# Boese0601/MagicDance

Measured on NVIDIA H100. Metric: denoise-steps/sec @512x512 50-step DDIM, higher is better.
Workload: dtype f16

## Files before the change

include/magicdance_b200.h:

```cpp
#ifndef MAGICDANCE_B200_H_
#define MAGICDANCE_B200_H_

#include <stdint.h>

#ifdef __cplusplus
extern "C" {
#endif

#define MDB_OK 0
#define MDB_ERR_INVALID (-1)
#define MDB_ERR_CUDA (-2)
#define MDB_ERR_UNSUPPORTED (-3)

#define MDB_ABI_VERSION 2

typedef void* mdb_stream_t;

int mdb_abi_version(void);
const char* mdb_last_error(void);
int mdb_device_check(void);
int64_t mdb_launch_count(void);
int64_t mdb_abi_struct_bytes(int32_t which);

#define MDB_TUNE_GEMM_PAIR_MIN_TILES 1
#define MDB_TUNE_ATTN40_2Q_MIN_CTAS 3
#define MDB_TUNE_GEMM_BN80_BELOW 4
enum {
  MDB_TUNE_GEMM_SKINNY_CTAS = 5,
  MDB_TUNE_GEMM_SPLIT_MIN_CHUNKS = 6
};
int mdb_set_tuning(int32_t key, int32_t value);
int32_t mdb_get_tuning(int32_t key);

#define MDB_EPI_NONE 0
#define MDB_EPI_GEGLU 1

typedef struct mdb_gemm_desc {
  const void* a;
  int64_t lda;
  const void* a2;
  int64_t lda2;
  int32_t k1;
  int32_t conv;
  int32_t nb, h, w, c;
  const void* b;
  int64_t ldb;
  void* d;
  int64_t ldd;
  const float* bias;
  int64_t bias_batch_stride;
  int32_t rows_per_batch;
  int32_t epilogue;
  const void* residual;
  int64_t ldr;
  int32_t m, n, k;
  int32_t splits;
  float* splitk_ws;
  const float* ln_u;
  float ln_eps;
} mdb_gemm_desc;

int mdb_gemm_f16(const mdb_gemm_desc* desc, mdb_stream_t stream);
// ... 148 lines not shown
```

magicdance_b200/_lib.py:

```python
from __future__ import annotations

import ctypes as C
import os

from . import build as _build

c_void_p, c_int32, c_int64, c_float = C.c_void_p, C.c_int32, C.c_int64, C.c_float


class GemmDesc(C.Structure):
    _fields_ = [
        ("a", c_void_p), ("lda", c_int64), ("a2", c_void_p), ("lda2", c_int64),
        ("k1", c_int32), ("conv", c_int32), ("nb", c_int32), ("h", c_int32), ("w", c_int32), ("c", c_int32),
        ("b", c_void_p), ("ldb", c_int64), ("d", c_void_p), ("ldd", c_int64),
        ("bias", c_void_p), ("bias_batch_stride", c_int64), ("rows_per_batch", c_int32), ("epilogue", c_int32),
        ("residual", c_void_p), ("ldr", c_int64),
        ("m", c_int32), ("n", c_int32), ("k", c_int32), ("splits", c_int32), ("splitk_ws", c_void_p),
        ("ln_u", c_void_p), ("ln_eps", c_float),
    ]


class AttnDesc(C.Structure):
    _fields_ = [
        ("q", c_void_p), ("ldq", c_int64),
# ... 102 lines not shown
    "mdb_layernorm_f16": (c_int32, [c_void_p, c_void_p, c_void_p, c_void_p, c_int64, c_int32, c_float, c_void_p]),
    "mdb_groupnorm_bwd_f16": (c_int32, [C.POINTER(GroupNormBwdDesc), c_void_p]),
    "mdb_groupnorm_bwd_ws_floats": (c_int64, [C.POINTER(GroupNormBwdDesc)]),
    "mdb_layernorm_bwd_f16": (c_int32, [C.POINTER(LayerNormBwdDesc), c_void_p]),
    "mdb_layernorm_bwd_ws_floats": (c_int64, [C.POINTER(LayerNormBwdDesc)]),
    "mdb_geglu_f16": (c_int32, [c_void_p, c_int64, c_void_p, c_int64, c_int64, c_int32, c_void_p]),
    "mdb_geglu_bwd_f16": (c_int32, [c_void_p, c_int64, c_void_p, c_int64, c_void_p, c_int64, c_int64, c_int32,
                                    c_void_p]),
    "mdb_conv3x3_direct_f16": (c_int32, [c_void_p, c_void_p, c_void_p, c_void_p, c_void_p, c_int32, c_int32, c_int32,
                                         c_int32, c_int32, c_int32, c_int32, c_void_p]),
    "mdb_conv3x3_direct_bwd_f16": (c_int32, [C.POINTER(Conv3x3BwdDesc), c_void_p]),
    "mdb_conv3x3_direct_bwd_ws_floats": (c_int64, [C.POINTER(Conv3x3BwdDesc)]),
    "mdb_im2col3x3_f16": (c_int32, [c_void_p, c_void_p, c_int32, c_int32, c_int32, c_int32, c_int32, c_void_p]),
    "mdb_im2col3x3_br_f16": (c_int32, [c_void_p, c_void_p, c_int32, c_int32, c_int32, c_int32, c_int32, c_void_p]),
    "mdb_upsample2x_f16": (c_int32, [c_void_p, c_void_p, c_int32, c_int32, c_int32, c_int32, c_void_p]),
    "mdb_upsample2x_bwd_f16": (c_int32, [c_void_p, c_void_p, c_int32, c_int32, c_int32, c_int32, c_int32, c_int32,
                                         c_void_p]),
    "mdb_add_f16": (c_int32, [c_void_p, c_void_p, c_void_p, c_int64, c_int32, c_int32, c_void_p]),
    "mdb_timestep_embedding_f32": (c_int32, [c_void_p, c_int32, c_void_p, c_int32, c_int32, c_void_p]),
    "mdb_skinny_linear_f32": (c_int32, [c_void_p, c_void_p, c_void_p, c_void_p, c_int32, c_int32, c_int32, c_int32,
                                        c_int32, c_void_p]),
    "mdb_skinny_linear_bwd_f32": (c_int32, [C.POINTER(SkinnyBwdDesc), c_void_p]),
    "mdb_skinny_linear_bwd_ws_floats": (c_int64, [C.POINTER(SkinnyBwdDesc)]),
    "mdb_nchw_f32_to_nhwc_f16": (c_int32, [c_void_p, c_void_p, c_int32, c_int32, c_int32, c_int32, c_int32, c_void_p]),
    "mdb_nhwc_f16_to_nchw_f32": (c_int32, [c_void_p, c_void_p, c_int32, c_int32, c_int32, c_int32, c_void_p]),
    "mdb_softmax_rows_f16": (c_int32, [c_void_p, c_int64, c_int32, c_int32, c_float, c_void_p]),
    "mdb_cfg_ddim_update_f32": (c_int32, [c_void_p, c_void_p, c_void_p, c_void_p, c_void_p, c_void_p, c_int64,
                                          c_void_p, c_int32, c_void_p]),
}

_lib = None
ABI_VERSION = 2
TUNE_GEMM_PAIR_MIN_TILES, TUNE_ATTN40_2Q_MIN_CTAS, TUNE_GEMM_BN80_BELOW = 1, 3, 4
TUNE_GEMM_SKINNY_CTAS, TUNE_GEMM_SPLIT_MIN_CHUNKS = 5, 6


def library_path() -> str:
    return os.environ.get("MAGICDANCE_B200_LIB", _build.LIB_PATH)


def load():
    global _lib
    if _lib is not None:
        return _lib
    path = library_path()
    if not os.path.isfile(path):
        raise RuntimeError(
            f"magicdance_b200: kernel library {path} is missing — run `python -m magicdance_b200.build` "
            "(there is no CPU/PyTorch fallback for the hot path)")
    if path == _build.LIB_PATH and os.path.isdir(_build.CSRC) and not _build.is_fresh():
        raise RuntimeError(f"magicdance_b200: {path} was not built from the sources in {_build.CSRC} "
                           "(stamp mismatch) — run `python -m magicdance_b200.build`")
    lib = C.CDLL(path)
    for name, (res, args) in SIGNATURES.items():
        fn = getattr(lib, name)
        fn.restype = res
        fn.argtypes = args
    if lib.mdb_abi_version() != ABI_VERSION:
        raise RuntimeError(f"magicdance_b200: ABI version mismatch ({lib.mdb_abi_version()} != {ABI_VERSION}); "
                           "rebuild the library")
    for which, mirror in ((0, GemmDesc), (1, AttnDesc), (2, AttnBwdDesc), (3, GemmBwdDesc), (4, GroupNormBwdDesc),
                          (5, LayerNormBwdDesc), (6, Conv3x3BwdDesc), (7, SkinnyBwdDesc)):
        if lib.mdb_abi_struct_bytes(which) != C.sizeof(mirror):
            raise RuntimeError(f"magicdance_b200: {mirror.__name__} mirrors {C.sizeof(mirror)} bytes, the library's "
                               f"struct has {lib.mdb_abi_struct_bytes(which)}: the binding and the library disagree")
    _lib = lib
    return lib
# ... 7 lines not shown
```

magicdance_b200/csrc/attention.cu:

```cuda
#include <stdlib.h>

#include <type_traits>

#include "common.cuh"

namespace mdb {

constexpr int kBQ = 128;

template <int D, int BKV, int STAGES>
struct AttnCfg {
  static constexpr int kDkChunks = (D + 63) / 64;
  static constexpr int kDV = (D + 15) / 16 * 16;
  static constexpr int kKSteps = kDV / 16;
  static constexpr int kQBytes = kDkChunks * kBQ * 128;
  static constexpr int kKBytes = kDkChunks * BKV * 128;
  static constexpr int kVBytes = kDV * 128;
  static constexpr int kStageBytes = kKBytes + kVBytes;
  static constexpr int kSmem = kQBytes + STAGES * kStageBytes + 1024;
  static_assert(BKV == 64, "one 128-byte swizzle row of keys per V^T tile");
  static_assert(kVBytes % 1024 == 0 && kKBytes % 1024 == 0, "stage tiles start on swizzle-atom boundaries");
};

struct AttnKParams {
// ... 142 lines not shown
    for (int h = 0; h < 2; ++h) {
      float l = l_run[h];
      l += __shfl_xor_sync(0xffffffffu, l, 1);
      l += __shfl_xor_sync(0xffffffffu, l, 2);
      inv_l[h] = 1.0f / l;
      l_row[h] = l;
    }
    const int r = wg * 64 + (warp & 3) * 16 + (lane >> 2);
    if constexpr (LSE) {
      if ((lane & 3) == 0) {
#pragma unroll
        for (int h = 0; h < 2; ++h) {
          const int q = q0 + r + 8 * h;
          if (q < p.nq)
            p.lse[(static_cast<long long>(b) * gridDim.y + head) * p.nq + q] =
                (m_run[h] + log2f(l_row[h])) * 0.6931471805599453f;
        }
      }
    }
#pragma unroll
    for (int h = 0; h < 2; ++h) {
      const int q = q0 + r + 8 * h;
      if (q < p.nq) {
        __half* op = p.out + (static_cast<long long>(b) * p.nq + q) * p.ldo + head * D + cq;
#pragma unroll
        for (int c8 = 0; c8 < D / 8; ++c8)
          *reinterpret_cast<uint32_t*>(op + 8 * c8) =
              pack_half2(o[4 * c8 + 2 * h] * inv_l[h], o[4 * c8 + 2 * h + 1] * inv_l[h]);
      }
    }
  }
}

static int g_attn40_2q_min_ctas = 512;
int get_attn_tuning() { return g_attn40_2q_min_ctas; }
void set_attn_tuning(int v) { g_attn40_2q_min_ctas = v; }

template <int D, int BKV, int STAGES, int MINB, bool LSE = false, typename P>
static int launch_attn(const P& kp, dim3 grid, cudaStream_t st) {
  using C = AttnCfg<D, BKV, STAGES>;
  static_assert(MINB == 1 || C::kSmem <= 113 * 1024, "two CTAs per SM must fit");
  constexpr auto kern = attn_wg_kernel<D, BKV, STAGES, MINB, LSE>;
  if (int rc = set_max_dyn_smem<kern>(C::kSmem)) return rc;
  MDB_CHECK_CUDA(launch_pdl(kern, grid, dim3(kWsThreads), C::kSmem, st, kp));
  count_launch();
  return MDB_OK;
}

template <int D, int BKV>
static int build_and_launch(const mdb_attn_desc* a, float* lse, cudaStream_t st) {
  constexpr int kDV = AttnCfg<D, BKV, 1>::kDV;
  AttnKParams kp;
  memset(&kp, 0, sizeof(kp));
  const int hd = a->heads * a->d;
  int rc;
  if ((rc = tmap_heads(&kp.tmQ, a->q, a->d, a->heads, (uint64_t)a->batch * a->nq, a->ldq, kBQ))) return rc;
  auto mk_kv = [&](const void* k, long long ldk, const void* vt, long long ldvt, int n, int nb, int ldvb,
                   CUtensorMap* tk, CUtensorMap* tv) -> int {
    int r = tmap_heads(tk, k, a->d, a->heads, (uint64_t)nb * n, ldk, BKV);
    if (r) return r;
    return tmap_vt(tv, vt, n, nb, ldvb, hd, ldvt, kDV);
  };
  if ((rc = mk_kv(a->k0, a->ldk0, a->vt0, a->ldvt0, a->n0, a->kv0_batches, a->ldv0_batch, &kp.tmK0, &kp.tmV0))) return rc;
  if (a->n1 > 0) {
    if ((rc = mk_kv(a->k1, a->ldk1, a->vt1, a->ldvt1, a->n1, a->kv1_batches, a->ldv1_batch, &kp.tmK1, &kp.tmV1)))
      return rc;
  }
  kp.out = static_cast<__half*>(a->out);
  kp.ldo = a->ldo;
  kp.nq = a->nq;
  kp.n0 = a->n0;
  kp.n1 = a->n1;
  kp.kv0_batches = a->kv0_batches;
  kp.kv1_batches = a->kv1_batches;
  kp.bank_batches = a->n1 > 0 ? a->bank_batches : 0;
  kp.scale_log2 = a->scale * 1.4426950408889634f;
  dim3 grid((a->nq + kBQ - 1) / kBQ, a->heads, a->batch);
  if (lse != nullptr) {
    AttnLseKParams lp;
    memset(&lp, 0, sizeof(lp));
    static_cast<AttnKParams&>(lp) = kp;
    lp.lse = lse;
    if constexpr (D == 40) {
      const long long ctas = (long long)grid.x * grid.y * grid.z;
      if (ctas >= (long long)g_attn40_2q_min_ctas) return launch_attn<D, BKV, 3, 2, true>(lp, grid, st);
    }
    return launch_attn<D, BKV, (D == 160 ? 2 : 4), 1, true>(lp, grid, st);
  }
  if constexpr (D == 40) {
    const long long ctas = (long long)grid.x * grid.y * grid.z;
    if (ctas >= (long long)g_attn40_2q_min_ctas) return launch_attn<D, BKV, 3, 2>(kp, grid, st);
  }
  return launch_attn<D, BKV, (D == 160 ? 2 : 4), 1>(kp, grid, st);
}

static int attention_entry(const mdb_attn_desc* a, float* lse, cudaStream_t st) {
  switch (a->d) {
    case 40:
      return build_and_launch<40, 64>(a, lse, st);
    case 80:
      return build_and_launch<80, 64>(a, lse, st);
    case 160:
      return build_and_launch<160, 64>(a, lse, st);
    default:
      set_error("mdb_attention_f16: head dim %d not supported (40, 80, 160)", a->d);
      return MDB_ERR_UNSUPPORTED;
  }
}

int attention_check_desc(const mdb_attn_desc* a) {
  MDB_REQUIRE(a != nullptr, "mdb_attention_f16: null descriptor");
  MDB_REQUIRE(a->q && a->k0 && a->vt0 && a->out, "mdb_attention_f16: null operand");
  MDB_REQUIRE(a->batch > 0 && a->heads > 0 && a->nq > 0 && a->n0 > 0 && a->n1 >= 0,
              "mdb_attention_f16: bad shape");
  MDB_REQUIRE(a->n1 == 0 || (a->k1 && a->vt1), "mdb_attention_f16: n1 > 0 needs k1/vt1");
  MDB_REQUIRE(a->kv0_batches == 1 || a->kv0_batches == a->batch, "mdb_attention_f16: kv0_batches must be 1 or batch");
  MDB_REQUIRE(a->n1 == 0 || a->kv1_batches == 1 || a->kv1_batches >= a->bank_batches,
              "mdb_attention_f16: kv1_batches must be 1 or cover bank_batches");
  MDB_REQUIRE(a->ldv0_batch >= a->n0 && a->ldv0_batch % 8 == 0, "mdb_attention_f16: ldv0_batch must be >= n0 and %% 8");
  MDB_REQUIRE(a->n1 == 0 || (a->ldv1_batch >= a->n1 && a->ldv1_batch % 8 == 0),
              "mdb_attention_f16: ldv1_batch must be >= n1 and %% 8");
  MDB_REQUIRE(a->ldo % 8 == 0 && (reinterpret_cast<uintptr_t>(a->out) & 15) == 0, "mdb_attention_f16: out alignment");
// ... 20 lines not shown
```

magicdance_b200/csrc/common.cuh:

```cuda
#pragma once

#include <cuda.h>
#include <cuda_fp16.h>
#include <cuda_runtime.h>
#include <cudaTypedefs.h>
#include <stdint.h>
#include <stdio.h>
#include <string.h>

#include "../../include/magicdance_b200.h"
#include "wgmma.cuh"

namespace mdb {

void set_error(const char* fmt, ...);

#define MDB_CHECK_CUDA(expr)                                                                     \
  do {                                                                                           \
    cudaError_t _e = (expr);                                                                     \
    if (_e != cudaSuccess) {                                                                     \
      mdb::set_error("%s:%d: %s failed: %s", __FILE__, __LINE__, #expr, cudaGetErrorString(_e)); \
      return MDB_ERR_CUDA;                                                                       \
    }                                                                                            \
  } while (0)

#define MDB_REQUIRE(cond, ...)      \
  do {                              \
    if (!(cond)) {                  \
      mdb::set_error(__VA_ARGS__);  \
      return MDB_ERR_INVALID;       \
    }                               \
  } while (0)

void count_launch(int n = 1);
int get_gemm_tuning(int key);
void set_gemm_tuning(int key, int value);
int get_attn_tuning();
void set_attn_tuning(int v);

constexpr int kNumSms = 132;

int tmap_rows(CUtensorMap* out, const void* base, uint64_t inner, uint64_t rows, long long ld, uint32_t box_inner,
              uint32_t box_rows);
int tmap_heads(CUtensorMap* out, const void* base, int d, int heads, uint64_t tokens, long long ld,
               uint32_t box_tokens);
int tmap_vt(CUtensorMap* out, const void* base, int n, int nb, long long ldvb, int rows, long long ldvt,
            uint32_t box_rows);
int tmap_nhwc(CUtensorMap* out, const void* base, int c, int w, int h, int nb, long long ld, const uint32_t box[4],
              int cs);
int tmap_nhwc_im2col(CUtensorMap* out, const void* base, int c, int w, int h, int nb, long long ld, int pixels,
                     int cs);

enum { kBoxOk, kBoxWideRows, kBoxRowsPerTile, kBoxImagesPerTile, kBoxTooLarge };
int pixel_box(int ho, int wo, int cs, int rows, bool fwd, uint32_t box[4]);

#ifdef __CUDACC__

bool pdl_enabled();
template <typename... KArgs, typename... Args>
inline cudaError_t launch_pdl_cluster2(void (*kernel)(KArgs...), dim3 grid, dim3 block, size_t smem,
                                       cudaStream_t stream, unsigned cluster_x, unsigned cluster_z, Args&&... args) {
  cudaLaunchConfig_t cfg;
  memset(&cfg, 0, sizeof(cfg));
  cfg.gridDim = grid;
  cfg.blockDim = block;
  cfg.dynamicSmemBytes = smem;
  cfg.stream = stream;
  cudaLaunchAttribute attr[2];
  int n = 0;
  if (cluster_z > 1 || cluster_x > 1) {
    attr[n].id = cudaLaunchAttributeClusterDimension;
// ... 255 lines not shown
```

magicdance_b200/csrc/misc.cu:

```cuda
#include <stdarg.h>
#include <stdlib.h>

#include <atomic>

#include "common.cuh"

namespace mdb {

static thread_local char g_err[512] = "";
static std::atomic<long long> g_launches{0};

void set_error(const char* fmt, ...) {
  va_list ap;
  va_start(ap, fmt);
  vsnprintf(g_err, sizeof(g_err), fmt, ap);
  va_end(ap);
}
void count_launch(int n) { g_launches.fetch_add(n, std::memory_order_relaxed); }
bool pdl_enabled() { return true; }

static PFN_cuTensorMapEncodeTiled_v12000 g_encode = nullptr;

static int make_tmap_f16(CUtensorMap* out, const void* base, int rank, const uint64_t* dims,
                         const uint64_t* strides_bytes, const uint32_t* box, const uint32_t* elem_strides = nullptr) {
// ... 524 lines not shown

extern "C" int64_t mdb_abi_struct_bytes(int32_t which) {
  switch (which) {
    case 0:
      return (int64_t)sizeof(mdb_gemm_desc);
    case 1:
      return (int64_t)sizeof(mdb_attn_desc);
    case 2:
      return (int64_t)sizeof(mdb_attn_bwd_desc);
    case 3:
      return (int64_t)sizeof(mdb_gemm_bwd_desc);
    case 4:
      return (int64_t)sizeof(mdb_groupnorm_bwd_desc);
    case 5:
      return (int64_t)sizeof(mdb_layernorm_bwd_desc);
    case 6:
      return (int64_t)sizeof(mdb_conv3x3_bwd_desc);
    case 7:
      return (int64_t)sizeof(mdb_skinny_linear_bwd_desc);
    default:
      return -1;
  }
}

extern "C" int mdb_set_tuning(int32_t key, int32_t value) {
  switch (key) {
    case MDB_TUNE_GEMM_PAIR_MIN_TILES:
    case MDB_TUNE_GEMM_BN80_BELOW:
    case MDB_TUNE_GEMM_SKINNY_CTAS:
    case MDB_TUNE_GEMM_SPLIT_MIN_CHUNKS:
      mdb::set_gemm_tuning(key, value);
      return MDB_OK;
    case MDB_TUNE_ATTN40_2Q_MIN_CTAS:
      mdb::set_attn_tuning(value);
      return MDB_OK;
    default:
      mdb::set_error("mdb_set_tuning: unknown key %d", key);
      return MDB_ERR_INVALID;
  }
}

extern "C" int32_t mdb_get_tuning(int32_t key) {
  if (key == MDB_TUNE_ATTN40_2Q_MIN_CTAS) return mdb::get_attn_tuning();
  return mdb::get_gemm_tuning(key);
}
extern "C" const char* mdb_last_error(void) { return mdb::g_err; }
extern "C" int64_t mdb_launch_count(void) { return mdb::g_launches.load(); }

extern "C" int mdb_device_check(void) {
  int dev = 0;
  MDB_CHECK_CUDA(cudaGetDevice(&dev));
  cudaDeviceProp prop;
  MDB_CHECK_CUDA(cudaGetDeviceProperties(&prop, dev));
  if (prop.major != 9 || prop.minor != 0) {
    set_error("device %d is sm_%d%d; this library is built for sm_90a only", dev, prop.major, prop.minor);
    return MDB_ERR_UNSUPPORTED;
  }
  return MDB_OK;
}

namespace {
__global__ void __launch_bounds__(256) softmax_rows_kernel(__half* __restrict__ x, long long ld, int cols, float scale_log2) {
  mdb::pdl_launch_dependents();
  mdb::pdl_wait();
  __shared__ float red[8];
  __shared__ float bcast;
  __half* row = x + static_cast<long long>(blockIdx.x) * ld;
  const int vecs = cols >> 3;
  const int lane = threadIdx.x & 31, warp = threadIdx.x >> 5;
  float m = -INFINITY;
  for (int v = threadIdx.x; v < vecs; v += blockDim.x) {
    const uint4 u = *reinterpret_cast<const uint4*>(row + v * 8);
    const __half2* h2 = reinterpret_cast<const __half2*>(&u);
#pragma unroll
    for (int e = 0; e < 4; ++e) {
      const float2 f = __half22float2(h2[e]);
// ... 213 lines not shown
```

magicdance_b200/csrc/wgmma.cuh:

```cuda
#pragma once
#include <stdint.h>

namespace mdb {

template <int N, int TA = 0, int TB = 0>
__device__ __forceinline__ void wgmma_ss(float (&d)[N / 2], uint64_t da, uint64_t db, uint32_t acc);
template <int N, int TB = 0>
__device__ __forceinline__ void wgmma_rs(float (&d)[N / 2], const uint32_t (&a)[4], uint64_t db, uint32_t acc);

template <>
__device__ __forceinline__ void wgmma_ss<64, 0, 0>(float (&d)[32], uint64_t da, uint64_t db, uint32_t acc) {
  asm volatile(
      "{\n\t.reg .pred p;\n\tsetp.ne.b32 p, %34, 0;\n\t"
      "wgmma.mma_async.sync.aligned.m64n64k16.f32.f16.f16 {%0, %1, %2, %3, %4, %5, %6, %7, %8, %9, %10, %11, %12, %13, %14, %15, %16, %17, %18, %19, %20, %21, %22, %23, %24, %25, %26, %27, %28, %29, %30, %31}, %32, %33, p, 1, 1, 0, 0;\n\t}"
      : "+f"(d[0]), "+f"(d[1]), "+f"(d[2]), "+f"(d[3]), "+f"(d[4]), "+f"(d[5]), "+f"(d[6]), "+f"(d[7]), "+f"(d[8]), "+f"(d[9]), "+f"(d[10]), "+f"(d[11]), "+f"(d[12]), "+f"(d[13]), "+f"(d[14]), "+f"(d[15]), "+f"(d[16]), "+f"(d[17]), "+f"(d[18]), "+f"(d[19]), "+f"(d[20]), "+f"(d[21]), "+f"(d[22]), "+f"(d[23]), "+f"(d[24]), "+f"(d[25]), "+f"(d[26]), "+f"(d[27]), "+f"(d[28]), "+f"(d[29]), "+f"(d[30]), "+f"(d[31])
      : "l"(da), "l"(db), "r"(acc));
}

template <>
__device__ __forceinline__ void wgmma_ss<80, 0, 0>(float (&d)[40], uint64_t da, uint64_t db, uint32_t acc) {
  asm volatile(
      "{\n\t.reg .pred p;\n\tsetp.ne.b32 p, %42, 0;\n\t"
      "wgmma.mma_async.sync.aligned.m64n80k16.f32.f16.f16 {%0, %1, %2, %3, %4, %5, %6, %7, %8, %9, %10, %11, %12, %13, %14, %15, %16, %17, %18, %19, %20, %21, %22, %23, %24, %25, %26, %27, %28, %29, %30, %31, %32, %33, %34, %35, %36, %37, %38, %39}, %40, %41, p, 1, 1, 0, 0;\n\t}"
      : "+f"(d[0]), "+f"(d[1]), "+f"(d[2]), "+f"(d[3]), "+f"(d[4]), "+f"(d[5]), "+f"(d[6]), "+f"(d[7]), "+f"(d[8]), "+f"(d[9]), "+f"(d[10]), "+f"(d[11]), "+f"(d[12]), "+f"(d[13]), "+f"(d[14]), "+f"(d[15]), "+f"(d[16]), "+f"(d[17]), "+f"(d[18]), "+f"(d[19]), "+f"(d[20]), "+f"(d[21]), "+f"(d[22]), "+f"(d[23]), "+f"(d[24]), "+f"(d[25]), "+f"(d[26]), "+f"(d[27]), "+f"(d[28]), "+f"(d[29]), "+f"(d[30]), "+f"(d[31]), "+f"(d[32]), "+f"(d[33]), "+f"(d[34]), "+f"(d[35]), "+f"(d[36]), "+f"(d[37]), "+f"(d[38]), "+f"(d[39])
// ... 34 lines not shown
      "wgmma.mma_async.sync.aligned.m64n64k16.f32.f16.f16 {%0, %1, %2, %3, %4, %5, %6, %7, %8, %9, %10, %11, %12, %13, %14, %15, %16, %17, %18, %19, %20, %21, %22, %23, %24, %25, %26, %27, %28, %29, %30, %31}, %32, %33, p, 1, 1, 0, 1;\n\t}"
      : "+f"(d[0]), "+f"(d[1]), "+f"(d[2]), "+f"(d[3]), "+f"(d[4]), "+f"(d[5]), "+f"(d[6]), "+f"(d[7]), "+f"(d[8]), "+f"(d[9]), "+f"(d[10]), "+f"(d[11]), "+f"(d[12]), "+f"(d[13]), "+f"(d[14]), "+f"(d[15]), "+f"(d[16]), "+f"(d[17]), "+f"(d[18]), "+f"(d[19]), "+f"(d[20]), "+f"(d[21]), "+f"(d[22]), "+f"(d[23]), "+f"(d[24]), "+f"(d[25]), "+f"(d[26]), "+f"(d[27]), "+f"(d[28]), "+f"(d[29]), "+f"(d[30]), "+f"(d[31])
      : "l"(da), "l"(db), "r"(acc));
}

template <>
__device__ __forceinline__ void wgmma_ss<64, 1, 0>(float (&d)[32], uint64_t da, uint64_t db, uint32_t acc) {
  asm volatile(
      "{\n\t.reg .pred p;\n\tsetp.ne.b32 p, %34, 0;\n\t"
      "wgmma.mma_async.sync.aligned.m64n64k16.f32.f16.f16 {%0, %1, %2, %3, %4, %5, %6, %7, %8, %9, %10, %11, %12, %13, %14, %15, %16, %17, %18, %19, %20, %21, %22, %23, %24, %25, %26, %27, %28, %29, %30, %31}, %32, %33, p, 1, 1, 1, 0;\n\t}"
      : "+f"(d[0]), "+f"(d[1]), "+f"(d[2]), "+f"(d[3]), "+f"(d[4]), "+f"(d[5]), "+f"(d[6]), "+f"(d[7]), "+f"(d[8]), "+f"(d[9]), "+f"(d[10]), "+f"(d[11]), "+f"(d[12]), "+f"(d[13]), "+f"(d[14]), "+f"(d[15]), "+f"(d[16]), "+f"(d[17]), "+f"(d[18]), "+f"(d[19]), "+f"(d[20]), "+f"(d[21]), "+f"(d[22]), "+f"(d[23]), "+f"(d[24]), "+f"(d[25]), "+f"(d[26]), "+f"(d[27]), "+f"(d[28]), "+f"(d[29]), "+f"(d[30]), "+f"(d[31])
      : "l"(da), "l"(db), "r"(acc));
}

template <>
__device__ __forceinline__ void wgmma_ss<128, 0, 1>(float (&d)[64], uint64_t da, uint64_t db, uint32_t acc) {
  asm volatile(
      "{\n\t.reg .pred p;\n\tsetp.ne.b32 p, %66, 0;\n\t"
      "wgmma.mma_async.sync.aligned.m64n128k16.f32.f16.f16 {%0, %1, %2, %3, %4, %5, %6, %7, %8, %9, %10, %11, %12, %13, %14, %15, %16, %17, %18, %19, %20, %21, %22, %23, %24, %25, %26, %27, %28, %29, %30, %31, %32, %33, %34, %35, %36, %37, %38, %39, %40, %41, %42, %43, %44, %45, %46, %47, %48, %49, %50, %51, %52, %53, %54, %55, %56, %57, %58, %59, %60, %61, %62, %63}, %64, %65, p, 1, 1, 0, 1;\n\t}"
      : "+f"(d[0]), "+f"(d[1]), "+f"(d[2]), "+f"(d[3]), "+f"(d[4]), "+f"(d[5]), "+f"(d[6]), "+f"(d[7]), "+f"(d[8]), "+f"(d[9]), "+f"(d[10]), "+f"(d[11]), "+f"(d[12]), "+f"(d[13]), "+f"(d[14]), "+f"(d[15]), "+f"(d[16]), "+f"(d[17]), "+f"(d[18]), "+f"(d[19]), "+f"(d[20]), "+f"(d[21]), "+f"(d[22]), "+f"(d[23]), "+f"(d[24]), "+f"(d[25]), "+f"(d[26]), "+f"(d[27]), "+f"(d[28]), "+f"(d[29]), "+f"(d[30]), "+f"(d[31]), "+f"(d[32]), "+f"(d[33]), "+f"(d[34]), "+f"(d[35]), "+f"(d[36]), "+f"(d[37]), "+f"(d[38]), "+f"(d[39]), "+f"(d[40]), "+f"(d[41]), "+f"(d[42]), "+f"(d[43]), "+f"(d[44]), "+f"(d[45]), "+f"(d[46]), "+f"(d[47]), "+f"(d[48]), "+f"(d[49]), "+f"(d[50]), "+f"(d[51]), "+f"(d[52]), "+f"(d[53]), "+f"(d[54]), "+f"(d[55]), "+f"(d[56]), "+f"(d[57]), "+f"(d[58]), "+f"(d[59]), "+f"(d[60]), "+f"(d[61]), "+f"(d[62]), "+f"(d[63])
      : "l"(da), "l"(db), "r"(acc));
}

template <>
__device__ __forceinline__ void wgmma_ss<128, 1, 1>(float (&d)[64], uint64_t da, uint64_t db, uint32_t acc) {
  asm volatile(
      "{\n\t.reg .pred p;\n\tsetp.ne.b32 p, %66, 0;\n\t"
      "wgmma.mma_async.sync.aligned.m64n128k16.f32.f16.f16 {%0, %1, %2, %3, %4, %5, %6, %7, %8, %9, %10, %11, %12, %13, %14, %15, %16, %17, %18, %19, %20, %21, %22, %23, %24, %25, %26, %27, %28, %29, %30, %31, %32, %33, %34, %35, %36, %37, %38, %39, %40, %41, %42, %43, %44, %45, %46, %47, %48, %49, %50, %51, %52, %53, %54, %55, %56, %57, %58, %59, %60, %61, %62, %63}, %64, %65, p, 1, 1, 1, 1;\n\t}"
      : "+f"(d[0]), "+f"(d[1]), "+f"(d[2]), "+f"(d[3]), "+f"(d[4]), "+f"(d[5]), "+f"(d[6]), "+f"(d[7]), "+f"(d[8]), "+f"(d[9]), "+f"(d[10]), "+f"(d[11]), "+f"(d[12]), "+f"(d[13]), "+f"(d[14]), "+f"(d[15]), "+f"(d[16]), "+f"(d[17]), "+f"(d[18]), "+f"(d[19]), "+f"(d[20]), "+f"(d[21]), "+f"(d[22]), "+f"(d[23]), "+f"(d[24]), "+f"(d[25]), "+f"(d[26]), "+f"(d[27]), "+f"(d[28]), "+f"(d[29]), "+f"(d[30]), "+f"(d[31]), "+f"(d[32]), "+f"(d[33]), "+f"(d[34]), "+f"(d[35]), "+f"(d[36]), "+f"(d[37]), "+f"(d[38]), "+f"(d[39]), "+f"(d[40]), "+f"(d[41]), "+f"(d[42]), "+f"(d[43]), "+f"(d[44]), "+f"(d[45]), "+f"(d[46]), "+f"(d[47]), "+f"(d[48]), "+f"(d[49]), "+f"(d[50]), "+f"(d[51]), "+f"(d[52]), "+f"(d[53]), "+f"(d[54]), "+f"(d[55]), "+f"(d[56]), "+f"(d[57]), "+f"(d[58]), "+f"(d[59]), "+f"(d[60]), "+f"(d[61]), "+f"(d[62]), "+f"(d[63])
      : "l"(da), "l"(db), "r"(acc));
}

template <>
__device__ __forceinline__ void wgmma_rs<48, 0>(float (&d)[24], const uint32_t (&a)[4], uint64_t db, uint32_t acc) {
  asm volatile(
      "{\n\t.reg .pred p;\n\tsetp.ne.b32 p, %29, 0;\n\t"
      "wgmma.mma_async.sync.aligned.m64n48k16.f32.f16.f16 {%0, %1, %2, %3, %4, %5, %6, %7, %8, %9, %10, %11, %12, %13, %14, %15, %16, %17, %18, %19, %20, %21, %22, %23}, {%24, %25, %26, %27}, %28, p, 1, 1, 0;\n\t}"
      : "+f"(d[0]), "+f"(d[1]), "+f"(d[2]), "+f"(d[3]), "+f"(d[4]), "+f"(d[5]), "+f"(d[6]), "+f"(d[7]), "+f"(d[8]), "+f"(d[9]), "+f"(d[10]), "+f"(d[11]), "+f"(d[12]), "+f"(d[13]), "+f"(d[14]), "+f"(d[15]), "+f"(d[16]), "+f"(d[17]), "+f"(d[18]), "+f"(d[19]), "+f"(d[20]), "+f"(d[21]), "+f"(d[22]), "+f"(d[23])
      : "r"(a[0]), "r"(a[1]), "r"(a[2]), "r"(a[3]), "l"(db), "r"(acc));
}

template <>
__device__ __forceinline__ void wgmma_rs<80, 0>(float (&d)[40], const uint32_t (&a)[4], uint64_t db, uint32_t acc) {
  asm volatile(
      "{\n\t.reg .pred p;\n\tsetp.ne.b32 p, %45, 0;\n\t"
      "wgmma.mma_async.sync.aligned.m64n80k16.f32.f16.f16 {%0, %1, %2, %3, %4, %5, %6, %7, %8, %9, %10, %11, %12, %13, %14, %15, %16, %17, %18, %19, %20, %21, %22, %23, %24, %25, %26, %27, %28, %29, %30, %31, %32, %33, %34, %35, %36, %37, %38, %39}, {%40, %41, %42, %43}, %44, p, 1, 1, 0;\n\t}"
      : "+f"(d[0]), "+f"(d[1]), "+f"(d[2]), "+f"(d[3]), "+f"(d[4]), "+f"(d[5]), "+f"(d[6]), "+f"(d[7]), "+f"(d[8]), "+f"(d[9]), "+f"(d[10]), "+f"(d[11]), "+f"(d[12]), "+f"(d[13]), "+f"(d[14]), "+f"(d[15]), "+f"(d[16]), "+f"(d[17]), "+f"(d[18]), "+f"(d[19]), "+f"(d[20]), "+f"(d[21]), "+f"(d[22]), "+f"(d[23]), "+f"(d[24]), "+f"(d[25]), "+f"(d[26]), "+f"(d[27]), "+f"(d[28]), "+f"(d[29]), "+f"(d[30]), "+f"(d[31]), "+f"(d[32]), "+f"(d[33]), "+f"(d[34]), "+f"(d[35]), "+f"(d[36]), "+f"(d[37]), "+f"(d[38]), "+f"(d[39])
      : "r"(a[0]), "r"(a[1]), "r"(a[2]), "r"(a[3]), "l"(db), "r"(acc));
}

template <>
__device__ __forceinline__ void wgmma_rs<160, 0>(float (&d)[80], const uint32_t (&a)[4], uint64_t db, uint32_t acc) {
  asm volatile(
      "{\n\t.reg .pred p;\n\tsetp.ne.b32 p, %85, 0;\n\t"
      "wgmma.mma_async.sync.aligned.m64n160k16.f32.f16.f16 {%0, %1, %2, %3, %4, %5, %6, %7, %8, %9, %10, %11, %12, %13, %14, %15, %16, %17, %18, %19, %20, %21, %22, %23, %24, %25, %26, %27, %28, %29, %30, %31, %32, %33, %34, %35, %36, %37, %38, %39, %40, %41, %42, %43, %44, %45, %46, %47, %48, %49, %50, %51, %52, %53, %54, %55, %56, %57, %58, %59, %60, %61, %62, %63, %64, %65, %66, %67, %68, %69, %70, %71, %72, %73, %74, %75, %76, %77, %78, %79}, {%80, %81, %82, %83}, %84, p, 1, 1, 0;\n\t}"
      : "+f"(d[0]), "+f"(d[1]), "+f"(d[2]), "+f"(d[3]), "+f"(d[4]), "+f"(d[5]), "+f"(d[6]), "+f"(d[7]), "+f"(d[8]), "+f"(d[9]), "+f"(d[10]), "+f"(d[11]), "+f"(d[12]), "+f"(d[13]), "+f"(d[14]), "+f"(d[15]), "+f"(d[16]), "+f"(d[17]), "+f"(d[18]), "+f"(d[19]), "+f"(d[20]), "+f"(d[21]), "+f"(d[22]), "+f"(d[23]), "+f"(d[24]), "+f"(d[25]), "+f"(d[26]), "+f"(d[27]), "+f"(d[28]), "+f"(d[29]), "+f"(d[30]), "+f"(d[31]), "+f"(d[32]), "+f"(d[33]), "+f"(d[34]), "+f"(d[35]), "+f"(d[36]), "+f"(d[37]), "+f"(d[38]), "+f"(d[39]), "+f"(d[40]), "+f"(d[41]), "+f"(d[42]), "+f"(d[43]), "+f"(d[44]), "+f"(d[45]), "+f"(d[46]), "+f"(d[47]), "+f"(d[48]), "+f"(d[49]), "+f"(d[50]), "+f"(d[51]), "+f"(d[52]), "+f"(d[53]), "+f"(d[54]), "+f"(d[55]), "+f"(d[56]), "+f"(d[57]), "+f"(d[58]), "+f"(d[59]), "+f"(d[60]), "+f"(d[61]), "+f"(d[62]), "+f"(d[63]), "+f"(d[64]), "+f"(d[65]), "+f"(d[66]), "+f"(d[67]), "+f"(d[68]), "+f"(d[69]), "+f"(d[70]), "+f"(d[71]), "+f"(d[72]), "+f"(d[73]), "+f"(d[74]), "+f"(d[75]), "+f"(d[76]), "+f"(d[77]), "+f"(d[78]), "+f"(d[79])
      : "r"(a[0]), "r"(a[1]), "r"(a[2]), "r"(a[3]), "l"(db), "r"(acc));
}

template <>
__device__ __forceinline__ void wgmma_rs<48, 1>(float (&d)[24], const uint32_t (&a)[4], uint64_t db, uint32_t acc) {
  asm volatile(
      "{\n\t.reg .pred p;\n\tsetp.ne.b32 p, %29, 0;\n\t"
      "wgmma.mma_async.sync.aligned.m64n48k16.f32.f16.f16 {%0, %1, %2, %3, %4, %5, %6, %7, %8, %9, %10, %11, %12, %13, %14, %15, %16, %17, %18, %19, %20, %21, %22, %23}, {%24, %25, %26, %27}, %28, p, 1, 1, 1;\n\t}"
      : "+f"(d[0]), "+f"(d[1]), "+f"(d[2]), "+f"(d[3]), "+f"(d[4]), "+f"(d[5]), "+f"(d[6]), "+f"(d[7]), "+f"(d[8]), "+f"(d[9]), "+f"(d[10]), "+f"(d[11]), "+f"(d[12]), "+f"(d[13]), "+f"(d[14]), "+f"(d[15]), "+f"(d[16]), "+f"(d[17]), "+f"(d[18]), "+f"(d[19]), "+f"(d[20]), "+f"(d[21]), "+f"(d[22]), "+f"(d[23])
      : "r"(a[0]), "r"(a[1]), "r"(a[2]), "r"(a[3]), "l"(db), "r"(acc));
// ... 22 lines not shown
```

magicdance_b200/ops.py:

```python
from __future__ import annotations

import ctypes as C
import os

import torch

from . import _lib

EPI_NONE, EPI_GEGLU = 0, 1
SKINNY_MAX_ROWS = 16
_GEMM_DEBUG = os.environ.get("MDB_GEMM_DEBUG", "0") == "1"
TRACE = None


class tuning:
    _KEYS = {"pair_min_tiles": _lib.TUNE_GEMM_PAIR_MIN_TILES,
             "attn40_2q_min_ctas": _lib.TUNE_ATTN40_2Q_MIN_CTAS, "bn80_below": _lib.TUNE_GEMM_BN80_BELOW,
             "skinny_ctas": _lib.TUNE_GEMM_SKINNY_CTAS, "split_min_chunks": _lib.TUNE_GEMM_SPLIT_MIN_CHUNKS}

    def __init__(self, **kw):
        self.want = {self._KEYS[k]: int(v) for k, v in kw.items() if v is not None}

    def __enter__(self):
        lib = _lib.load()
        self.old = {k: int(lib.mdb_get_tuning(k)) for k in self.want}
        for k, v in self.want.items():
            _lib.check(lib.mdb_set_tuning(k, v), "set_tuning")
        return self

    def __exit__(self, *a):
        lib = _lib.load()
        for k, v in self.old.items():
            lib.mdb_set_tuning(k, v)


def _stream() -> int:
    return torch.cuda.current_stream().cuda_stream


def _ptr(t):
    return None if t is None else t.data_ptr()


def _chk(t: torch.Tensor, dtype, name):
    if not t.is_cuda:
        raise RuntimeError(f"magicdance_b200: {name} must be a CUDA tensor (no CPU fallback exists for the hot path)")
    if t.dtype != dtype:
        raise RuntimeError(f"magicdance_b200: {name} must be {dtype}, got {t.dtype}")


def require_cuda(device):
# ... 1038 lines not shown
```

Before: 93.31.

## Add warp-specialized pipelined attention kernel for head dim 40

Adds a new attention kernel for head dimension 40 with a dedicated TMA producer warp and four consumer warpgroups that share a 6-stage K/V ring. Each step overlaps the previous tile's P·V wgmma with the current tile's QK^T and softmax. It also adds an m64n40k16 register-A wgmma specialization and a tuning key that selects this kernel, on by default. Phase-reduced variants (modes 2 and 3) skip work and are kept for probing. The aim is to hide softmax latency and memory loads behind tensor-core work in the D=40 self-attention layers. The cost is higher register pressure and one CTA per SM.

After: 94.85 (median of 6 runs). +1.7%, better.

```diff
diff --git a/include/magicdance_b200.h b/include/magicdance_b200.h
--- a/include/magicdance_b200.h
+++ b/include/magicdance_b200.h
@@ -27,7 +27,8 @@
 #define MDB_TUNE_GEMM_BN80_BELOW 4
 enum {
   MDB_TUNE_GEMM_SKINNY_CTAS = 5,
-  MDB_TUNE_GEMM_SPLIT_MIN_CHUNKS = 6
+  MDB_TUNE_GEMM_SPLIT_MIN_CHUNKS = 6,
+  MDB_TUNE_ATTN40_PIPE = 8
 };
 int mdb_set_tuning(int32_t key, int32_t value);
 int32_t mdb_get_tuning(int32_t key);
diff --git a/magicdance_b200/_lib.py b/magicdance_b200/_lib.py
--- a/magicdance_b200/_lib.py
+++ b/magicdance_b200/_lib.py
@@ -158,7 +158,7 @@
 _lib = None
 ABI_VERSION = 2
 TUNE_GEMM_PAIR_MIN_TILES, TUNE_ATTN40_2Q_MIN_CTAS, TUNE_GEMM_BN80_BELOW = 1, 3, 4
-TUNE_GEMM_SKINNY_CTAS, TUNE_GEMM_SPLIT_MIN_CHUNKS = 5, 6
+TUNE_GEMM_SKINNY_CTAS, TUNE_GEMM_SPLIT_MIN_CHUNKS, TUNE_ATTN40_PIPE = 5, 6, 8
 
 
 def library_path() -> str:
diff --git a/magicdance_b200/csrc/attention.cu b/magicdance_b200/csrc/attention.cu
--- a/magicdance_b200/csrc/attention.cu
+++ b/magicdance_b200/csrc/attention.cu
@@ -198,9 +198,204 @@
   }
 }
 
+template <int NWG>
+struct Attn40PipeCfg {
+  static constexpr int kBQ = 64 * NWG;
+  static constexpr int kThreads = 128 * NWG + 32;
+  static constexpr int kQBytes = kBQ * 128;
+  static_assert(NWG % 2 == 0, "Q arrives in 128-row TMA boxes");
+};
+
+template <int STAGES, int NWG, int MINB, int PHASES = 3>
+__global__ void __launch_bounds__(Attn40PipeCfg<NWG>::kThreads, MINB)
+    attn40_pipe_kernel(const __grid_constant__ AttnKParams p) {
+  constexpr int D = 40, BKV = 64;
+  using C = AttnCfg<D, BKV, STAGES>;
+  using PC = Attn40PipeCfg<NWG>;
+  constexpr int kProducer = 4 * NWG;
+  extern __shared__ uint8_t smem_raw[];
+  __shared__ __align__(8) uint64_t q_bar;
+  __shared__ __align__(8) uint64_t kv_full[STAGES], kv_empty[STAGES];
+
+  uint8_t* sQ = align1024(smem_raw);
+  uint8_t* sKV = sQ + PC::kQBytes;
+
+  const int warp = threadIdx.x >> 5;
+  const int lane = threadIdx.x & 31;
+  const int q0 = blockIdx.x * PC::kBQ;
+  const int head = blockIdx.y;
+  const int b = blockIdx.z;
+  const int t0 = (p.n0 + BKV - 1) / BKV;
+  const int t1 = (b < p.bank_batches && p.n1 > 0) ? (p.n1 + BKV - 1) / BKV : 0;
+  const int n_tiles = t0 + t1;
+
+  pdl_launch_dependents();
+  if (warp == kProducer && lane == 0) {
+    tma_prefetch_desc(&p.tmQ);
+    tma_prefetch_desc(&p.tmK0);
+    tma_prefetch_desc(&p.tmV0);
+    mbar_init(&q_bar, 1);
+    for (int s = 0; s < STAGES; ++s) {
+      mbar_init(&kv_full[s], 1);
+      mbar_init(&kv_empty[s], 128 * NWG);
+    }
+    fence_barrier_init();
+  }
+  __syncthreads();
+  pdl_wait();
+
+  if (warp == kProducer) {
+    if (lane == 0) {
+      mbar_expect_tx(&q_bar, PC::kQBytes);
+      for (int i = 0; i < NWG / 2; ++i)
+        tma_load_3d(sQ + i * (128 * 128), &p.tmQ, &q_bar, 0, head, b * p.nq + q0 + 128 * i);
+      for (int j = 0; j < n_tiles; ++j) {
+        const bool src1 = j >= t0;
+        const int key0 = (src1 ? (j - t0) : j) * BKV;
+        const CUtensorMap* tk = src1 ? &p.tmK1 : &p.tmK0;
+        const CUtensorMap* tv = src1 ? &p.tmV1 : &p.tmV0;
+        const int nsrc = src1 ? p.n1 : p.n0;
+        const int kvb = src1 ? (p.kv1_batches > 1 ? b : 0) : (p.kv0_batches > 1 ? b : 0);
+        const int s = ring_acquire<STAGES>(kv_empty, j);
+        mbar_expect_tx(&kv_full[s], C::kStageBytes);
+        uint8_t* sk = sKV + s * C::kStageBytes;
+        tma_load_3d(sk, tk, &kv_full[s], 0, head, kvb * nsrc + key0);
+        tma_load_3d(sk + C::kKBytes, tv, &kv_full[s], key0, kvb, head * D);
+      }
+    }
+    return;
+  }
+
+  const int wg = warp >> 2;
+  const uint32_t q_addr = smem_u32(sQ) + wg * (64 * 128);
+  const int cq = 2 * (lane & 3);
+  float o[D / 2];
+#pragma unroll
+  for (int i = 0; i < D / 2; ++i) o[i] = 0.f;
+  float m_run[2] = {-INFINITY, -INFINITY};
+  float l_run[2] = {0.f, 0.f};
+  float sc[BKV / 2];
+  uint32_t pa[BKV / 16][4];
+  int s_prev = 0;
+  auto v_addr = [&](int st) { return smem_u32(sKV + st * C::kStageBytes + C::kKBytes); };
+  mbar_wait(&q_bar, 0);
+
+  auto step = [&](const int j, auto pv_tag) {
+    constexpr bool PV = decltype(pv_tag)::value;
+    const bool src1 = j >= t0;
+    const int key0 = (src1 ? (j - t0) : j) * BKV;
+    const int valid = min(BKV, (src1 ? p.n1 : p.n0) - key0);
+    const int s = ring_wait_full<STAGES>(kv_full, j);
+    const uint32_t k_addr = smem_u32(sKV + s * C::kStageBytes);
+
+    wgmma_fence();
+#pragma unroll
+    for (int ks = 0; ks < C::kKSteps; ++ks)
+      wgmma_ss<BKV>(sc, wgmma_desc_k_sw128(q_addr) + 2 * ks, wgmma_desc_k_sw128(k_addr) + 2 * ks, ks != 0 ? 1u : 0u);
+    wgmma_commit();
+    if constexpr (PV) {
+#pragma unroll
+      for (int kk = 0; kk < BKV / 16; ++kk) wgmma_rs<D>(o, pa[kk], wgmma_desc_k_sw128(v_addr(s_prev)) + 2 * kk, 1u);
+      wgmma_commit();
+    }
+    if constexpr (PV)
+      wgmma_wait<1>();
+    else
+      wgmma_wait<0>();
+    wgmma_fence_regs(sc);
+
+    float alpha[2] = {1.f, 1.f};
+    (void)alpha;
+    if constexpr (PHASES >= 2) {
+      if (valid < BKV) {
+#pragma unroll
+        for (int i = 0; i < BKV / 2; ++i)
+          if (8 * (i >> 2) + cq + (i & 1) >= valid) sc[i] = -INFINITY;
+      }
+      float mx[2] = {-INFINITY, -INFINITY};
+#pragma unroll
+      for (int i = 0; i < BKV / 2; ++i) mx[(i >> 1) & 1] = fmaxf(mx[(i >> 1) & 1], sc[i]);
+      float neg_m[2];
+#pragma unroll
+      for (int h = 0; h < 2; ++h) {
+        mx[h] = fmaxf(mx[h], __shfl_xor_sync(0xffffffffu, mx[h], 1));
+        mx[h] = fmaxf(mx[h], __shfl_xor_sync(0xffffffffu, mx[h], 2));
+        const float m_new = fmaxf(m_run[h], mx[h] * p.scale_log2);
+        alpha[h] = ex2_approx(m_run[h] - m_new);
+        m_run[h] = m_new;
+        neg_m[h] = -m_new;
+      }
+      float ls[2] = {0.f, 0.f};
+#pragma unroll
+      for (int i = 0; i < BKV / 2; i += 2) {
+        const int h = (i >> 1) & 1;
+        sc[i] = ex2_approx(fmaf(sc[i], p.scale_log2, neg_m[h]));
+        sc[i + 1] = ex2_approx(fmaf(sc[i + 1], p.scale_log2, neg_m[h]));
+        ls[h] += sc[i] + sc[i + 1];
+      }
+#pragma unroll
+      for (int h = 0; h < 2; ++h) l_run[h] = fmaf(l_run[h], alpha[h], ls[h]);
+    }
+
+    if constexpr (PV) {
+      wgmma_wait<0>();
+      wgmma_fence_regs(o);
+#pragma unroll
+      for (int kk = 0; kk < BKV / 16; ++kk)
+#pragma unroll
+        for (int e = 0; e < 4; ++e) asm volatile("" : "+r"(pa[kk][e])::"memory");
+      mbar_arrive(&kv_empty[s_prev]);
+    }
+    if constexpr (PHASES == 3) {
+#pragma unroll
+      for (int i = 0; i < D / 2; ++i) o[i] *= alpha[(i >> 1) & 1];
+#pragma unroll
+      for (int i = 0; i < BKV / 2; i += 2) pa[i >> 3][(i >> 1) & 3] = pack_half2(sc[i], sc[i + 1]);
+    } else {
+#pragma unroll
+      for (int i = 0; i < BKV / 2; ++i) asm volatile("" ::"f"(sc[i]));
+      mbar_arrive(&kv_empty[s]);
+    }
+    s_prev = s;
+  };
+  step(0, std::false_type());
+  for (int j = 1; j < n_tiles; ++j) step(j, std::integral_constant<bool, PHASES == 3>());
+  if constexpr (PHASES == 3) {
+    wgmma_fence();
+#pragma unroll
+    for (int kk = 0; kk < BKV / 16; ++kk) wgmma_rs<D>(o, pa[kk], wgmma_desc_k_sw128(v_addr(s_prev)) + 2 * kk, 1u);
+    wgmma_commit();
+    wgmma_wait<0>();
+    wgmma_fence_regs(o);
+    mbar_arrive(&kv_empty[s_prev]);
+  }
+
+  float inv_l[2];
+#pragma unroll
+  for (int h = 0; h < 2; ++h) {
+    float l = l_run[h];
+    l += __shfl_xor_sync(0xffffffffu, l, 1);
+    l += __shfl_xor_sync(0xffffffffu, l, 2);
+    inv_l[h] = 1.0f / l;
+  }
+  const int r = wg * 64 + (warp & 3) * 16 + (lane >> 2);
+#pragma unroll
+  for (int h = 0; h < 2; ++h) {
+    const int q = q0 + r + 8 * h;
+    if (q < p.nq) {
+      __half* op = p.out + (static_cast<long long>(b) * p.nq + q) * p.ldo + head * D + cq;
+#pragma unroll
+      for (int c8 = 0; c8 < D / 8; ++c8)
+        *reinterpret_cast<uint32_t*>(op + 8 * c8) =
+            pack_half2(o[4 * c8 + 2 * h] * inv_l[h], o[4 * c8 + 2 * h + 1] * inv_l[h]);
+    }
+  }
+}
+
 static int g_attn40_2q_min_ctas = 512;
-int get_attn_tuning() { return g_attn40_2q_min_ctas; }
-void set_attn_tuning(int v) { g_attn40_2q_min_ctas = v; }
+static int g_attn40_pipe = 1;
+int get_attn_tuning(int key) { return key == MDB_TUNE_ATTN40_PIPE ? g_attn40_pipe : g_attn40_2q_min_ctas; }
+void set_attn_tuning(int key, int v) { (key == MDB_TUNE_ATTN40_PIPE ? g_attn40_pipe : g_attn40_2q_min_ctas) = v; }
 
 template <int D, int BKV, int STAGES, int MINB, bool LSE = false, typename P>
 static int launch_attn(const P& kp, dim3 grid, cudaStream_t st) {
@@ -209,6 +404,19 @@
   constexpr auto kern = attn_wg_kernel<D, BKV, STAGES, MINB, LSE>;
   if (int rc = set_max_dyn_smem<kern>(C::kSmem)) return rc;
   MDB_CHECK_CUDA(launch_pdl(kern, grid, dim3(kWsThreads), C::kSmem, st, kp));
+  count_launch();
+  return MDB_OK;
+}
+
+template <int STAGES, int NWG, int MINB, int PHASES = 3>
+static int launch_attn40_pipe(const AttnKParams& kp, int nq, int heads, int batch, cudaStream_t st) {
+  using PC = Attn40PipeCfg<NWG>;
+  constexpr int kSmem = PC::kQBytes + STAGES * AttnCfg<40, 64, STAGES>::kStageBytes + 1024;
+  static_assert(kSmem * MINB <= 227 * 1024, "the CTAs of an SM must fit");
+  constexpr auto kern = attn40_pipe_kernel<STAGES, NWG, MINB, PHASES>;
+  if (int rc = set_max_dyn_smem<kern>(kSmem)) return rc;
+  const dim3 grid((nq + PC::kBQ - 1) / PC::kBQ, heads, batch);
+  MDB_CHECK_CUDA(launch_pdl(kern, grid, dim3(PC::kThreads), kSmem, st, kp));
   count_launch();
   return MDB_OK;
 }
@@ -254,6 +462,12 @@
     return launch_attn<D, BKV, (D == 160 ? 2 : 4), 1, true>(lp, grid, st);
   }
   if constexpr (D == 40) {
+    switch (g_attn40_pipe) {
+      case 1: return launch_attn40_pipe<6, 4, 1>(kp, a->nq, a->heads, a->batch, st);
+      case 2: return launch_attn40_pipe<6, 4, 1, 1>(kp, a->nq, a->heads, a->batch, st);
+      case 3: return launch_attn40_pipe<6, 4, 1, 2>(kp, a->nq, a->heads, a->batch, st);
+      default: break;
+    }
     const long long ctas = (long long)grid.x * grid.y * grid.z;
     if (ctas >= (long long)g_attn40_2q_min_ctas) return launch_attn<D, BKV, 3, 2>(kp, grid, st);
   }
diff --git a/magicdance_b200/csrc/common.cuh b/magicdance_b200/csrc/common.cuh
--- a/magicdance_b200/csrc/common.cuh
+++ b/magicdance_b200/csrc/common.cuh
@@ -35,8 +35,8 @@
 void count_launch(int n = 1);
 int get_gemm_tuning(int key);
 void set_gemm_tuning(int key, int value);
-int get_attn_tuning();
-void set_attn_tuning(int v);
+int get_attn_tuning(int key);
+void set_attn_tuning(int key, int v);
 
 constexpr int kNumSms = 132;
 
diff --git a/magicdance_b200/csrc/misc.cu b/magicdance_b200/csrc/misc.cu
--- a/magicdance_b200/csrc/misc.cu
+++ b/magicdance_b200/csrc/misc.cu
@@ -580,7 +580,8 @@
       mdb::set_gemm_tuning(key, value);
       return MDB_OK;
     case MDB_TUNE_ATTN40_2Q_MIN_CTAS:
-      mdb::set_attn_tuning(value);
+    case MDB_TUNE_ATTN40_PIPE:
+      mdb::set_attn_tuning(key, value);
       return MDB_OK;
     default:
       mdb::set_error("mdb_set_tuning: unknown key %d", key);
@@ -589,7 +590,7 @@
 }
 
 extern "C" int32_t mdb_get_tuning(int32_t key) {
-  if (key == MDB_TUNE_ATTN40_2Q_MIN_CTAS) return mdb::get_attn_tuning();
+  if (key == MDB_TUNE_ATTN40_2Q_MIN_CTAS || key == MDB_TUNE_ATTN40_PIPE) return mdb::get_attn_tuning(key);
   return mdb::get_gemm_tuning(key);
 }
 extern "C" const char* mdb_last_error(void) { return mdb::g_err; }
diff --git a/magicdance_b200/csrc/wgmma.cuh b/magicdance_b200/csrc/wgmma.cuh
--- a/magicdance_b200/csrc/wgmma.cuh
+++ b/magicdance_b200/csrc/wgmma.cuh
@@ -90,6 +90,15 @@
 }
 
 template <>
+__device__ __forceinline__ void wgmma_rs<40, 0>(float (&d)[20], const uint32_t (&a)[4], uint64_t db, uint32_t acc) {
+  asm volatile(
+      "{\n\t.reg .pred p;\n\tsetp.ne.b32 p, %25, 0;\n\t"
+      "wgmma.mma_async.sync.aligned.m64n40k16.f32.f16.f16 {%0, %1, %2, %3, %4, %5, %6, %7, %8, %9, %10, %11, %12, %13, %14, %15, %16, %17, %18, %19}, {%20, %21, %22, %23}, %24, p, 1, 1, 0;\n\t}"
+      : "+f"(d[0]), "+f"(d[1]), "+f"(d[2]), "+f"(d[3]), "+f"(d[4]), "+f"(d[5]), "+f"(d[6]), "+f"(d[7]), "+f"(d[8]), "+f"(d[9]), "+f"(d[10]), "+f"(d[11]), "+f"(d[12]), "+f"(d[13]), "+f"(d[14]), "+f"(d[15]), "+f"(d[16]), "+f"(d[17]), "+f"(d[18]), "+f"(d[19])
+      : "r"(a[0]), "r"(a[1]), "r"(a[2]), "r"(a[3]), "l"(db), "r"(acc));
+}
+
+template <>
 __device__ __forceinline__ void wgmma_rs<48, 0>(float (&d)[24], const uint32_t (&a)[4], uint64_t db, uint32_t acc) {
   asm volatile(
       "{\n\t.reg .pred p;\n\tsetp.ne.b32 p, %29, 0;\n\t"
diff --git a/magicdance_b200/ops.py b/magicdance_b200/ops.py
--- a/magicdance_b200/ops.py
+++ b/magicdance_b200/ops.py
@@ -16,7 +16,8 @@
 class tuning:
     _KEYS = {"pair_min_tiles": _lib.TUNE_GEMM_PAIR_MIN_TILES,
              "attn40_2q_min_ctas": _lib.TUNE_ATTN40_2Q_MIN_CTAS, "bn80_below": _lib.TUNE_GEMM_BN80_BELOW,
-             "skinny_ctas": _lib.TUNE_GEMM_SKINNY_CTAS, "split_min_chunks": _lib.TUNE_GEMM_SPLIT_MIN_CHUNKS}
+             "skinny_ctas": _lib.TUNE_GEMM_SKINNY_CTAS, "split_min_chunks": _lib.TUNE_GEMM_SPLIT_MIN_CHUNKS,
+             "attn40_pipe": _lib.TUNE_ATTN40_PIPE}
 
     def __init__(self, **kw):
         self.want = {self._KEYS[k]: int(v) for k, v in kw.items() if v is not None}
```
